# GloireLINVANI/3D_Gaussian_Splatting_Project

Hardware: AMD Instinct MI355X
Metric: Gaussians·views/sec labelled (3M G, 1080p), majority vote; first vote_view submit -> labels on the host (higher is better)
Workload: dtype f64

## Files before the change

### 3d_gaussian_splatting_project_amd/csrc/gsx_api.cpp

```cpp
#include <cstring>
#include <exception>
#include <new>

#include "gsx_ctx.hpp"

namespace gsx {

static thread_local std::string g_err;

void set_global_error(const char* fmt, ...) {
    char buf[512];
    va_list ap;
    va_start(ap, fmt);
    vsnprintf(buf, sizeof buf, fmt, ap);
    va_end(ap);
    g_err = buf;
}

int fail(Ctx* c, int code, const char* fmt, ...) {
    char buf[768];
    va_list ap;
    va_start(ap, fmt);
    vsnprintf(buf, sizeof buf, fmt, ap);
    va_end(ap);
// ... 155 lines not shown
    }
    else if (k == "render_multi_pre") c->opt_render_multi_pre = value != 0;
    else if (k == "render_bin32") c->opt_render_bin32 = value != 0;
    else if (k == "render_compact") c->opt_render_compact = value != 0;
    else if (k == "render_wide_sort") c->opt_render_wide_sort = value < 0 ? 0 : (value > 2 ? 2 : (int)value);
    else if (k == "render_share_stream") {
        if ((value != 0) != (c->opt_render_share_stream != 0)) gsx::render_release_twin(c);
        c->opt_render_share_stream = value != 0;
    }
    else if (k == "render_frames") {
        if (value < 1 || value > Ctx::kMaxFrames) return gsx::fail(c, GSX_E_INVALID, "set_option: render_frames must be in [1,%d]", (int)Ctx::kMaxFrames);
        c->opt_render_frames = (int)value;
    }
    else if (k == "blend_pk2") c->opt_blend_pk2 = value < 0 ? 0 : (value > 2 ? 2 : (int)value);
    else if (k == "exchange_slabs") {
        if (value < 1 || value > 64) return gsx::fail(c, GSX_E_INVALID, "set_option: exchange_slabs must be in [1,64]");
        c->opt_slabs = (int)value;
    } else if (k == "exchange_local") c->opt_local_codes = value != 0;
    else if (k == "flat_project") c->opt_flat_project = value != 0;
    else if (k == "seg_coarse") c->opt_seg_coarse = value != 0;
    else if (k == "batched_counts") c->opt_batched_counts = value != 0;
    else if (k == "wave_cull") c->opt_wave_cull = value != 0;
    else if (k == "filter_project") c->opt_filter_project = value != 0;
    else if (k == "host_pack") c->opt_host_pack = value != 0;
    else if (k == "labels_u8") c->opt_labels_u8 = value != 0;
    else if (k == "host_compact") c->opt_host_compact = value != 0;
    else if (k == "early_vote") {
        if (value < 0 || value > 2) return gsx::fail(c, GSX_E_INVALID, "set_option: early_vote must be 0, 1 or 2");
        c->opt_early_vote = (int)value;
    } else if (k == "early_replay") c->opt_early_replay = value != 0;
    else if (k == "early_vote_at") {
        if (value < 0 || value > 1000) return gsx::fail(c, GSX_E_INVALID, "set_option: early_vote_at must be in [0,1000] (permille of the announced views; 0 = from the hand-over rate)");
        c->opt_early_at = (int)value;
    }
    else if (k == "host_prefetch") gsx::set_host_prefetch((int)value);
    else if (k == "host_prefetch_burst") gsx::set_host_prefetch_burst(value != 0);
#ifdef GSX_EXPERIMENTS
    else if (k == "ablate") c->opt_ablate = (int)value;
#endif
    else if (k == "host_threads") {
        if (value < 0 || value > 256) return gsx::fail(c, GSX_E_INVALID, "set_option: host_threads must be in [0,256]");
        if ((int)value != c->opt_host_threads) {
            delete c->workers;
            c->workers = nullptr;
        }
        c->opt_host_threads = (int)value;
    }
    else if (k == "vote_unroll") {
        if (value != 2 && value != 4 && value != 8)
            return gsx::fail(c, GSX_E_INVALID, "set_option: vote_unroll must be 2, 4 or 8");
        c->opt_vote_unroll = (int)value;
    } else
        return gsx::fail(c, GSX_E_INVALID, "set_option: unknown option '%s'", name);
    return GSX_OK;
}

int gsx_get_option(gsx_ctx* ctx, const char* name, int64_t* value) {
    CTX_OR_FAIL(ctx);
    if (!name || !value) return gsx::fail(c, GSX_E_INVALID, "get_option: NULL argument");
    const std::string k(name);
    if (k == "early_vote") *value = c->opt_early_vote;
    else if (k == "early_vote_at") *value = c->opt_early_at;
    else if (k == "early_replay") *value = c->opt_early_replay ? 1 : 0;
    else if (k == "seg_tiled") *value = c->opt_seg_tiled ? 1 : 0;
    else if (k == "seg_coarse") *value = c->opt_seg_coarse ? 1 : 0;
    else
// ... 750 lines not shown
```

### 3d_gaussian_splatting_project_amd/csrc/gsx_ctx.hpp

```cpp
#pragma once
#include <hip/hip_runtime.h>

#include <chrono>
#include <cstdarg>
#include <cstdint>
#include <cstdio>
#include <map>
#include <cstddef>
#include <string>
#include <vector>

#include "../../include/gsx.h"
#include "host_pack.hpp"

namespace gsx {

void set_global_error(const char* fmt, ...);
struct Ctx;
int fail(Ctx* c, int code, const char* fmt, ...);

#define GSX_HIP(ctx, call)                                                                         \
    do {                                                                                           \
        hipError_t e__ = (call);                                                                   \
        if (e__ != hipSuccess)                                                                     \
// ... 161 lines not shown
    void* h_scratch = nullptr;
    size_t h_scratch_cap = 0;
    long long compact_bytes = 0;
    void* h_labels = nullptr;
    size_t h_labels_cap = 0;
    hipEvent_t h_ev[kLabelChunks] = {nullptr, nullptr, nullptr, nullptr};
    void* h_views = nullptr;
    size_t h_views_cap = 0;
    hipEvent_t h_views_ev = nullptr;
    std::vector<ViewDesc> own_views;
    int own_first_view = 0;
    const void* pool_base = nullptr;
    int n_flushed = 0;
    bool planes_valid = false;
    bool planes_zero = false;
    bool planes_stale = false;
    DevBuf cnt, fv;
    DevBuf keys, labels;
    DevBuf labels8;
    DevBuf bcnt, bcodes;
    DevBuf cand, codes;
    long long counts_n = -1, counts_npad = -1, counts_sn = -1, codes_n = -1, codes_npad = -1;
    int counts_bins = -1;
    bool labels_valid = false;
    int opt_filter_project = 1;
    int opt_early_vote = 1;
    int opt_early_at = 0;
    std::chrono::steady_clock::time_point early_t0;
    int opt_early_replay = 1;
    bool early_replayed = false;
    int early_state = 0;
    int early_done = 0;
    int early_batches = 0;
    hipStream_t stream2 = nullptr;
    bool stream_borrowed = false;
    int opt_render_share_stream = 1;
    bool early_inflight = false;
    hipEvent_t early_maps_ev = nullptr, early_done_ev = nullptr, early_up_ev = nullptr;
    DevBuf ecnt, efv;
    DevBuf erec;
    DevBuf e_views, e_cull;
    void* h_early = nullptr;
    size_t h_early_cap = 0;

    int64_t rn = 0;
    DevBuf r_order, r_buffer, r_tex;
    DevBuf r_sh;
    DevBuf r_fdc, r_shc;
    bool r_sh_valid = false, r_sh_on = false;
    int r_sh_deg = 0;
    DevBuf r_labels, r_edit_code, r_edit_tab, r_edit_hidden;
    bool r_edits_on = false;
    int64_t r_edit_hidden_n = 0;
    DevBuf r_image;
    int r_W = 0, r_H = 0;
    DevBuf r_ranges, r_small, r_scan;
    DevBuf r_depth, r_bucket, r_rect, r_count, r_offset, r_rec;
    DevBuf r_pre;
    struct PreSet {
        DevBuf depth, rect, rec, pre;
    };
    static constexpr int kPreSets = 3;
    PreSet r_sets[kPreSets];
    DevBuf r_pre_args;
    std::vector<unsigned long long> r_pre_args_host;
    hipEvent_t r_pre_ev[kPreSets] = {nullptr, nullptr, nullptr};
// ... 156 lines not shown
```

### 3d_gaussian_splatting_project_amd/csrc/vote.hip

```cpp
#include <hip/hip_runtime.h>

#include <chrono>
#include <cmath>

#include <algorithm>
#include <cmath>
#include <cstdlib>
#include <cstring>
#include <new>

#include <type_traits>

#include "gsx_ctx.hpp"

namespace gsx {

static constexpr int kBlock = 256;
static constexpr int kMaxBatch = 255;
int early_join(Ctx* c);

struct ViewRegs {
    double R[9], t[3], fx, fy, half_w, half_h, width, height;
    long long seg_off;
    int seg_w, unit_scale, seg_row_bytes, cam_w, cam_h;
// ... 490 lines not shown
    const double Z = valid ? (double)p.z[i] : 0.0;
    const uint8_t* __restrict__ pool = p.pool;

    int best = -1;
    int bestc = 0;
    const CullMasks cmask = wave_cull_masks(p.cull, p.cull_pitch, p.nviews, X, Y, Z, p.cull_tally);
    auto chunk = [&](auto full, int vb) {
        constexpr bool kFull = decltype(full)::value;
        int bin[U];
        gather_chunk<U, DIV, kFull>(views, pool, vb, X, Y, Z, cull_bits<U>(cmask, p.nviews - vb), bin, p.filt_h);
#pragma unroll
        for (int u = 0; u < U; ++u) {
            if (bin[u] >= 0) {
                const int c = h[bin[u]] + 1;
                h[bin[u]] = (uint8_t)c;
                if (c >= bestc) {
                    bestc = c;
                    best = bin[u];
                }
            }
        }
        };
    int vb = p.nviews;
    for (; vb >= U; vb -= U) chunk(std::true_type{}, vb);
    if (vb > 0) chunk(std::false_type{}, vb);
    if (valid) {
        const long long o = p.perm ? (long long)p.perm[i] : i;
        labels[o] = best - 1 + (best < 0);
    }
}

template <int U, int DIV>
__global__ __launch_bounds__(kBlock) void vote_record_kernel(FusedParams p, const ViewDesc* __restrict__ views,
                                                             uint8_t* __restrict__ rec) {
    const long long i = (long long)logical_block(blockIdx.x, gridDim.x, p.xcd_swizzle) * kBlock + threadIdx.x;
    const bool valid = i < p.n;
    const long long ic = valid ? i : 0;
    const float xf = p.x[ic], yf = p.y[ic], zf = p.z[ic];
    const double X = valid ? (double)xf : __builtin_nan("");
    const double Y = valid ? (double)yf : 0.0;
    const double Z = valid ? (double)zf : 0.0;
    const uint8_t* __restrict__ pool = p.pool;
    const int lane = threadIdx.x & 63;
    uint8_t* r = rec + (i - lane) * p.nviews + lane;
    const CullMasks cmask = wave_cull_masks(p.cull, p.cull_pitch, p.nviews, X, Y, Z, p.cull_tally);
    auto chunk = [&](auto full, int vb) {
        constexpr bool kFull = decltype(full)::value;
        int bin[U];
        gather_chunk<U, DIV, kFull>(views, pool, vb, X, Y, Z, cull_bits<U>(cmask, p.nviews - vb), bin, p.filt_h);
#pragma unroll
        for (int u = 0; u < U; ++u)
            if (kFull || vb - 1 - u >= 0) r[(vb - 1 - u) * 64] = (uint8_t)(bin[u] + 1);
    };
    int vb = p.nviews;
    for (; vb >= U; vb -= U) chunk(std::true_type{}, vb);
    if (vb > 0) chunk(std::false_type{}, vb);
}

template <int U, int DIV>
__global__ __launch_bounds__(kBlock) void vote_fused_replay_kernel(FusedParams p, const ViewDesc* __restrict__ views,
                                                                   const uint8_t* __restrict__ rec, int E,
                                                                   int* __restrict__ labels) {
    extern __shared__ uint32_t lds[];
    uint32_t* row = lds + threadIdx.x * p.stride_dw;
    uint8_t* h = reinterpret_cast<uint8_t*>(row);
    for (int k = 0; k < p.stride_dw; ++k) row[k] = 0;
    const long long i = (long long)logical_block(blockIdx.x, gridDim.x, p.xcd_swizzle) * kBlock + threadIdx.x;
    const bool valid = i < p.n;
    const long long ic = valid ? i : 0;
    const float xf = p.x[ic], yf = p.y[ic], zf = p.z[ic];
    const double X = valid ? (double)xf : __builtin_nan("");
    const double Y = valid ? (double)yf : 0.0;
    const double Z = valid ? (double)zf : 0.0;
    const uint8_t* __restrict__ pool = p.pool;
    int best = -1, bestc = 0;
    auto vote = [&](int b) {
        const int c = h[b] + 1;
        h[b] = (uint8_t)c;
        if (c >= bestc) {
            bestc = c;
            best = b;
        }
    };
    const CullMasks cmask = wave_cull_masks(p.cull, p.cull_pitch, p.nviews, X, Y, Z, p.cull_tally);
    auto chunk = [&](auto full, int vb) {
        constexpr bool kFull = decltype(full)::value;
        int bin[U];
        gather_chunk<U, DIV, kFull>(views, pool, vb, X, Y, Z, cull_bits<U>(cmask, p.nviews - vb), bin, p.filt_h);
#pragma unroll
        for (int u = 0; u < U; ++u)
            if (bin[u] >= 0) vote(bin[u]);
    };
    int vb = p.nviews;
    for (; vb >= U; vb -= U) chunk(std::true_type{}, vb);
    if (vb > 0) chunk(std::false_type{}, vb);
    constexpr int kReplay = 16;
    const int lane = threadIdx.x & 63;
    const uint8_t* __restrict__ r = rec + (i - lane) * E + lane;
    for (int v0 = E; v0 > 0; v0 -= kReplay) {
        unsigned b[kReplay];
#pragma unroll
        for (int j = 0; j < kReplay; ++j) {
            const int v = v0 - 1 - j;
            const unsigned got = r[max(v, 0) * 64];
            b[j] = v >= 0 ? got : 0u;
        }
#pragma unroll
        for (int j = 0; j < kReplay; ++j)
            if (b[j]) vote((int)b[j] - 1);
    }
    if (valid) {
        const long long o = p.perm ? (long long)p.perm[i] : i;
        labels[o] = best - 1 + (best < 0);
    }
}

typedef unsigned short u16x2 __attribute__((ext_vector_type(2)));
__device__ __forceinline__ uint32_t pk_max_u16(uint32_t a, uint32_t b) {
    return __builtin_bit_cast(uint32_t, __builtin_elementwise_max(__builtin_bit_cast(u16x2, a), __builtin_bit_cast(u16x2, b)));
}

template <int U, int DIV, int NQ>
__global__ __launch_bounds__(kBlock, 4) void vote_fused_final_kernel(FusedParams p, const ViewDesc* __restrict__ views,
                                                                     const uint8_t* __restrict__ cntA,
                                                                     const uint8_t* __restrict__ fvA,
                                                                     const uint8_t* __restrict__ recA, int E,
                                                                     int* __restrict__ labels, int ablate_arg) {
#ifdef GSX_EXPERIMENTS
    const int ablate = ablate_arg;
#else
    constexpr int ablate = 0;
// ... 508 lines not shown
        return fail(c, GSX_E_UNSUPPORTED, "vote_begin: n_classes=%d outside [1,255] (u8 seg maps)", n_classes);
    if (first_view < 0 || total_views < 1 || total_views > 65535 || first_view >= total_views)
        return fail(c, GSX_E_INVALID, "vote_begin: first_view=%d total_views=%d (need 0 <= first < total <= 65535)",
                    first_view, total_views);
    GSX_HIP(c, hipSetDevice(c->device));
    c->n_classes = n_classes;
    c->bins = n_classes + 1;
    c->first_view = first_view;
    c->total_views = total_views;
    c->local_codes = c->opt_local_codes != 0;
    c->wide = total_views > 255 && !c->local_codes;
    c->slabs = c->opt_slabs > 0 ? c->opt_slabs : 1;
    c->sn = ((c->n + c->slabs - 1) / c->slabs + 255) / 256 * 256;
    if (c->sn == 0) c->sn = 256;
    c->n_pad = c->sn * c->slabs;
    c->views.clear();
    c->pend_count = 0;
    c->compact_bytes = 0;
    c->views_dirty = true;
    c->pool_base = nullptr;
    c->seg_used = 0;
    c->n_flushed = 0;
    c->planes_valid = false;
    c->planes_zero = false;
    c->planes_stale = false;
    c->labels_valid = false;
    {
        const int rcj = early_join(c);
        if (rcj) return rcj;
    }
    c->early_state = 0;
    c->early_done = 0;
    c->early_batches = 0;
    GSX_HIP(c, c->errflag.ensure(sizeof(int)));
    GSX_HIP(c, hipMemsetAsync(c->errflag.p, 0x7f, sizeof(int), c->stream));
    c->vote_begun = true;
    return GSX_OK;
}

static int pool_reserve(Ctx* c, size_t need) {
    if (need <= c->segpool.cap) return GSX_OK;
    {
        const int rcf = vote_flush_pending(c);
        if (rcf) return rcf;
    }
    if (c->early_state == 1 || c->early_batches > 0) {
        GSX_HIP(c, hipStreamSynchronize(c->stream2));
        c->early_inflight = false;
        c->early_state = -1;
        c->early_batches = 0;
    }
    size_t cap = c->segpool.cap ? c->segpool.cap : ((size_t)64 << 20);
    while (cap < need) cap *= 2;
    void* np = nullptr;
    GSX_HIP(c, hipMalloc(&np, cap));
    if (c->seg_used) {
        hipError_t e = hipMemcpyAsync(np, c->segpool.p, c->seg_used, hipMemcpyDeviceToDevice, c->stream);
        if (e == hipSuccess) e = hipStreamSynchronize(c->stream);
        if (e != hipSuccess) {
            (void)hipFree(np);
            return fail(c, GSX_E_HIP, "seg pool growth copy failed: %s", hipGetErrorString(e));
        }
    }
    c->segpool.release();
    c->segpool.p = np;
    c->segpool.cap = cap;
// ... 26 lines not shown
        const size_t all = stride * (size_t)(c->total_views - c->first_view);
        need = std::max(need, std::min(all, (size_t)32 << 30));
    }
    return pool_reserve(c, need);
}

static void push_view(Ctx* c, const gsx_camera* cam, const MapLayout& L, size_t off, int img_w, int img_h) {
    ViewDesc vd;
    fill_view_desc(vd, cam, L.w, L.h, img_w, img_h);
    vd.seg_off = (long long)off;
    vd.seg_row_bytes = L.strip_bytes;
    vd.coarse_row_bytes = L.cstrip_bytes;
    vd.coarse_delta = (unsigned)L.coarse_off;
    c->views.push_back(vd);
    c->views_dirty = true;
    c->seg_used = off + L.map_bytes;
    c->labels_valid = false;
}

static void launch_pack(Ctx* c, const PackArgs& a, int jobs, int seg_dtype, bool vec, long long cells);

static Workers* host_workers(Ctx* c, const void* near = nullptr) {
    if (!c->workers) {
        try {
            c->workers = new Workers(c->opt_host_threads > 0 ? c->opt_host_threads : default_host_threads(), numa_node_of(near));
        } catch (...) {
            c->workers = nullptr;
        }
    }
    return c->workers;
}

static int early_vote_stage(Ctx* c);

static int vote_view_host(Ctx* c, const gsx_camera* cam, const void* seg, int seg_dtype, int seg_w, int seg_h, int img_w, int img_h) {
    MapLayout L;
    int rc = view_prologue(c, "vote_view", cam, seg, 1, seg_dtype, seg_w, seg_h, img_w, img_h, L);
    if (rc) return rc;
    if (c->opt_host_pack) {
        const size_t stride = (L.map_bytes + 255) / 256 * 256;
        constexpr int kSlots = kDmaBatch * kDmaGroups;
        const bool compact = c->opt_host_compact && L.strip_bytes && L.cstrip_bytes;
        const CompactLayout CL = compact ? compact_layout(L) : CompactLayout{};
        const size_t slot_bytes = compact ? (CL.capacity + 255) / 256 * 256 : stride;
        if (c->hring_slot != slot_bytes || !c->hring || c->hring_compact != compact) {
            if ((rc = vote_flush_pending(c))) return rc;
            for (int g = 0; g < kDmaGroups; ++g) {
                if (c->hring_busy[g]) GSX_HIP(c, hipEventSynchronize(c->hring_ev[g]));
                c->hring_busy[g] = false;
                if (!c->hring_ev[g]) GSX_HIP(c, hipEventCreateWithFlags(&c->hring_ev[g], hipEventDisableTiming));
            }
            if (c->hring_bytes < slot_bytes * kSlots) {
                if (c->hring) GSX_HIP(c, hipHostFree(c->hring));
                c->hring = nullptr;
                c->hring_bytes = 0;
                GSX_HIP(c, hipHostMalloc(&c->hring, slot_bytes * kSlots, hipHostMallocDefault));
                c->hring_bytes = slot_bytes * kSlots;
            }
            if (!compact) std::memset(c->hring, 0, slot_bytes * kSlots);
            c->hring_slot = slot_bytes;
            c->hring_compact = compact;
            c->hring_next = 0;
            c->cgrp = 0;
            c->grp_recs = 0;
        }
        const size_t off = (c->seg_used + 255) / 256 * 256;
// ... 86 lines not shown
        if (slot.cap < raw) {
            GSX_HIP(c, hipHostFree(slot.p));
            slot.p = nullptr;
            slot.cap = 0;
            GSX_HIP(c, hipHostMalloc(&slot.p, raw, hipHostMallocDefault));
            slot.cap = raw;
        }
        DevBuf& land = c->dstage[c->ring_next];
        GSX_HIP(c, land.ensure(raw));
        host_copy(host_workers(c, seg), slot.p, seg, raw);
        GSX_HIP(c, hipMemcpyAsync(land.p, slot.p, raw, hipMemcpyHostToDevice, c->stream));
        const size_t off = (c->seg_used + 255) / 256 * 256;
        PackArgs a{};
        a.src[0] = land.p;
        a.dst[0] = c->segpool.as<uint8_t>() + off;
        a.view[0] = c->first_view + (int)c->views.size();
        a.w = L.w, a.h = L.h, a.strip_bytes = L.strip_bytes, a.cstrip_bytes = L.cstrip_bytes, a.cw = L.cw, a.ch = L.ch;
        a.bins = c->bins;
        a.coarse_off = (unsigned)L.coarse_off;
        a.err = c->errflag.as<int>();
        launch_pack(c, a, 1, seg_dtype, seg_w % 4 == 0, (long long)L.cw * L.ch);
        GSX_HIP(c, hipGetLastError());
        GSX_HIP(c, hipEventRecord(slot.ev, c->stream));
        slot.busy = true;
        c->ring_next = (c->ring_next + 1) % kPinSlots;
        push_view(c, cam, L, off, img_w, img_h);
        return GSX_OK;
    }
    return GSX_OK;
}

int vote_view(Ctx* c, const gsx_camera* cam, const void* seg, int seg_dtype, int seg_w, int seg_h, int img_w, int img_h) {
    const int rc = vote_view_host(c, cam, seg, seg_dtype, seg_w, seg_h, img_w, img_h);
    return rc ? rc : early_vote_stage(c);
}

static void launch_pack(Ctx* c, const PackArgs& a, int jobs, int seg_dtype, bool vec, long long cells) {
    using K = void (*)(PackArgs);
    static const K table[4][2] = {{seg_pack_fused_kernel<int32_t, 1, false>, seg_pack_fused_kernel<int32_t, 1, true>},
                                  {seg_pack_fused_kernel<int64_t, 1, false>, seg_pack_fused_kernel<int64_t, 1, true>},
                                  {seg_pack_fused_kernel<uint8_t, 0, false>, seg_pack_fused_kernel<uint8_t, 0, true>},
                                  {seg_pack_fused_kernel<uint8_t, 1, false>, seg_pack_fused_kernel<uint8_t, 1, true>}};
    ProfScope ps(c, "seg_pack");
    hipLaunchKernelGGL(table[seg_dtype][vec ? 1 : 0], dim3(grid_for(cells), jobs), dim3(kBlock), 0, c->stream, a);
}

int vote_views_device(Ctx* c, int n, const gsx_camera* cams, const void* const* segs, int seg_dtype, int seg_w, int seg_h,
                      int img_w, int img_h) {
    if (n <= 0) return n == 0 ? GSX_OK : fail(c, GSX_E_INVALID, "vote_views_device: n < 0");
    MapLayout L;
    int rc = view_prologue(c, "vote_views_device", cams, segs, n, seg_dtype, seg_w, seg_h, img_w, img_h, L);
    if (rc) return rc;
    for (int i = 0; i < n; ++i)
        if (!segs[i]) return fail(c, GSX_E_INVALID, "vote_views_device: map %d is NULL", i);
    const size_t esz = seg_dtype == GSX_SEG_I32 ? 4 : seg_dtype == GSX_SEG_I64 ? 8 : 1;
    const long long cells = (long long)L.cw * L.ch;
    for (int i0 = 0; i0 < n; i0 += kPackBatch) {
        const int m = std::min(kPackBatch, n - i0);
        PackArgs a{};
        bool vec = seg_w % 4 == 0;
        size_t off = 0;
        for (int k = 0; k < m; ++k) {
            off = (c->seg_used + 255) / 256 * 256;
            a.src[k] = segs[i0 + k];
            a.dst[k] = c->segpool.as<uint8_t>() + off;
            a.view[k] = c->first_view + (int)c->views.size();
            vec = vec && reinterpret_cast<uintptr_t>(segs[i0 + k]) % (4 * esz) == 0;
            push_view(c, cams + i0 + k, L, off, img_w, img_h);
        }
        a.w = L.w, a.h = L.h, a.strip_bytes = L.strip_bytes, a.cstrip_bytes = L.cstrip_bytes, a.cw = L.cw, a.ch = L.ch;
        a.bins = c->bins;
        a.coarse_off = (unsigned)L.coarse_off;
        a.err = c->errflag.as<int>();
        launch_pack(c, a, m, seg_dtype, vec, cells);
        GSX_HIP(c, hipGetLastError());
    }
    return GSX_OK;
}

int vote_flush_pending(Ctx* c) {
    if (!c->pend_count) return GSX_OK;
    GSX_HIP(c, hipSetDevice(c->device));
    if (c->hring_compact) {
        const int g = c->pend_group;
        const size_t gcap = (size_t)kDmaBatch * c->hring_slot;
        GSX_HIP(c, c->cstage.ensure(gcap));
        const uint8_t* src = static_cast<uint8_t*>(c->hring) + (size_t)g * gcap;
        if (!(c->opt_ablate & 1))
            GSX_HIP(c, hipMemcpyAsync(c->cstage.as<uint8_t>() + c->pend_lo, src + c->pend_lo, c->grp_used - c->pend_lo, hipMemcpyHostToDevice,
                                      c->stream));
        GSX_HIP(c, hipEventRecord(c->hring_ev[g], c->stream));
        c->hring_busy[g] = true;
        const MapLayout& L = c->pend_L;
        const CompactLayout CL = compact_layout(L);
        ExpandArgs a{};
        for (int k = 0; k < c->pend_count; ++k) {
            a.rec[k] = c->cstage.as<uint8_t>() + c->pend_rec[k];
            a.map[k] = c->segpool.as<uint8_t>() + c->pend_map[k];
        }
        a.w = L.w, a.h = L.h, a.strip_bytes = L.strip_bytes, a.cstrip_bytes = L.cstrip_bytes, a.cw = L.cw, a.ch = L.ch;
        a.strips = (L.w + 15) / 16;
        a.table_bytes = (unsigned)CL.table_bytes, a.stream_off = (unsigned)CL.stream_off, a.coarse_off = (unsigned)L.coarse_off;
        a.fine_bytes = (unsigned)L.fine_bytes, a.map_bytes = (unsigned)L.map_bytes, a.stride = (unsigned)((L.map_bytes + 255) / 256 * 256);
        a.max_block = (unsigned)(L.cw - 1);
        if (!(c->opt_ablate & 3)) {
            ProfScope ps(c, "seg_expand");
            hipLaunchKernelGGL(seg_expand_kernel, dim3((unsigned)CL.bands, (unsigned)c->pend_count), dim3(kBlock), 0, c->stream, a);
            GSX_HIP(c, hipGetLastError());
// ... 295 lines not shown
}

int vote_rewind(Ctx* c) {
    if (!c->vote_begun) return fail(c, GSX_E_STATE, "vote_rewind before vote_begin");
    GSX_HIP(c, hipSetDevice(c->device));
    c->n_flushed = 0;
    c->labels_valid = false;
    c->early_state = -1;
    c->early_batches = 0;
    {
        const int rcj = early_join(c);
        if (rcj) return rcj;
    }
    if (c->planes_valid) {
        c->planes_valid = false;
        c->planes_zero = false;
        c->planes_stale = true;
    }
    return GSX_OK;
}

template <class K>
static int set_lds(Ctx* c, K kernel, size_t bytes) {
    if (bytes > 160 * 1024) return fail(c, GSX_E_UNSUPPORTED, "vote: %zu B of LDS per workgroup exceeds 160 KiB", bytes);
    GSX_HIP(c, hipFuncSetAttribute(reinterpret_cast<const void*>(kernel), hipFuncAttributeMaxDynamicSharedMemorySize,
                                   (int)bytes));
    return GSX_OK;
}

static constexpr int kUnroll = 8;

FusedParams fused_params(Ctx* c, int stride_bytes_per_bin);
static constexpr int kEarlyPitch = 256;
static constexpr long long kEarlyMinGaussians = 1 << 18;
static constexpr int kEarlyMinViews = 32;
static constexpr double kEarlyUsPerGaussianView = 4.4e-6;
static constexpr double kRecordUsPerGaussianView = 1.7e-6;
static constexpr size_t kEarlySlack = 64 * 260;
static constexpr size_t kEarlyCullDoubles = (size_t)kCullStride * kCullPlanes * kEarlyPitch;

static bool early_common(const Ctx* c) {
    return c->opt_early_vote && c->first_view == 0 && !c->local_codes && c->slabs == 1 && c->n_flushed == 0 && !c->pool_base &&
           c->opt_flat_project && c->n > 0 && c->bins <= 255 &&
           (c->opt_early_vote == 2 || (c->n >= kEarlyMinGaussians && c->total_views >= kEarlyMinViews));
}
static bool early_possible(const Ctx* c) { return early_common(c) && c->total_views <= kMaxBatch && !c->wide; }
static bool early_batched_possible(const Ctx* c) { return early_common(c) && c->total_views > kMaxBatch && c->opt_batched_counts; }
static int early_batch_stage(Ctx* c);
static int early_batch_count(int total) {
    const int tail = std::min(std::max(total / 16, 16), 64), body = total - tail;
    return (body + kMaxBatch - 1) / kMaxBatch + 1;
}
static void early_batch_bounds(int total, int s, int& lo, int& hi) {
    const int tail = std::min(std::max(total / 16, 16), 64), body = total - tail;
    const int Sb = (body + kMaxBatch - 1) / kMaxBatch;
    if (s >= Sb) {
        lo = body;
        hi = total;
    } else {
        lo = (int)((long long)body * s / Sb);
        hi = (int)((long long)body * (s + 1) / Sb);
    }
}

static int early_upload(Ctx* c, int lo, int hi, int block, int blocks, hipStream_t st, int* dm) {
    const size_t vbytes = sizeof(ViewDesc) * kEarlyPitch, cbytes = sizeof(double) * kEarlyCullDoubles;
    if (!c->h_early) {
        GSX_HIP(c, hipHostMalloc(&c->h_early, vbytes + cbytes, hipHostMallocDefault));
        c->h_early_cap = vbytes + cbytes;
    }
    GSX_HIP(c, c->e_views.ensure(sizeof(ViewDesc) * (size_t)std::max(kEarlyPitch, c->total_views)));
    GSX_HIP(c, c->e_cull.ensure(cbytes * (size_t)std::max(2, blocks)));
    if (!c->early_up_ev) GSX_HIP(c, hipEventCreateWithFlags(&c->early_up_ev, hipEventDisableTiming));
    else GSX_HIP(c, hipEventSynchronize(c->early_up_ev));
    ViewDesc* hv = static_cast<ViewDesc*>(c->h_early);
    double* planes = reinterpret_cast<double*>(static_cast<char*>(c->h_early) + vbytes);
    std::memset(planes, 0, cbytes);
    const long long base = (long long)reinterpret_cast<uintptr_t>(c->segpool.p);
    bool simple = true, coarse = true;
    for (int i = lo; i < hi; ++i) {
        ViewDesc& v = hv[i - lo];
        v = c->views[i];
        v.seg_off += base;
        simple = simple && v.unit_scale && v.seg_row_bytes;
        coarse = coarse && v.coarse_row_bytes;
        double pl[kCullStride * kCullPlanes];
        cull_planes(v, pl);
        for (int k = 0; k < kCullStride * kCullPlanes; ++k) planes[(size_t)k * kEarlyPitch + (i - lo)] = pl[k];
    }
    *dm = flat_div_mode(c, simple, coarse);
    if (hi > lo) GSX_HIP(c, hipMemcpyAsync(c->e_views.as<ViewDesc>() + lo, hv, sizeof(ViewDesc) * (size_t)(hi - lo), hipMemcpyHostToDevice, st));
    GSX_HIP(c, hipMemcpyAsync(c->e_cull.as<double>() + (size_t)block * kEarlyCullDoubles, planes, cbytes, hipMemcpyHostToDevice, st));
    GSX_HIP(c, hipEventRecord(c->early_up_ev, st));
    return GSX_OK;
}

static FusedParams early_params(Ctx* c, int lo, int hi, int block, int stride_bytes_per_bin) {
    FusedParams p = fused_params(c, stride_bytes_per_bin);
    p.views = c->e_views.as<ViewDesc>() + lo;
    p.nviews = hi - lo;
    p.cull = c->opt_wave_cull ? c->e_cull.as<double>() + (size_t)block * kEarlyCullDoubles : nullptr;
    p.cull_pitch = kEarlyPitch;
    return p;
}

int early_join(Ctx* c) {
    if (!c->early_inflight) return GSX_OK;
    GSX_HIP(c, hipStreamWaitEvent(c->stream, c->early_done_ev, 0));
    c->early_inflight = false;
    return GSX_OK;
}

int second_stream(Ctx* c) {
    if (c->stream2) return GSX_OK;
    int least = 0, greatest = 0;
    GSX_HIP(c, hipDeviceGetStreamPriorityRange(&least, &greatest));
    GSX_HIP(c, hipStreamCreateWithPriority(&c->stream2, hipStreamNonBlocking, least));
    return GSX_OK;
}

static int early_streams(Ctx* c) {
    const int rc = second_stream(c);
    if (rc) return rc;
    if (!c->early_maps_ev) GSX_HIP(c, hipEventCreateWithFlags(&c->early_maps_ev, hipEventDisableTiming));
    if (!c->early_done_ev) GSX_HIP(c, hipEventCreateWithFlags(&c->early_done_ev, hipEventDisableTiming));
    return GSX_OK;
}

static int early_vote_stage(Ctx* c) {
    if (c->early_state == 0 && early_batched_possible(c)) return early_batch_stage(c);
    if (c->early_state != 0 || !early_possible(c)) return GSX_OK;
    const int nv = (int)c->views.size();
    int at;
    if (c->opt_early_at > 0) {
        at = std::max(1, (int)(((long long)c->total_views * c->opt_early_at + 999) / 1000));
        if (nv != at) return GSX_OK;
    } else {
        const auto now = std::chrono::steady_clock::now();
        if (nv == 1) c->early_t0 = now;
        if (nv < std::max(8, c->total_views / 4)) return GSX_OK;
        const double t_map = std::chrono::duration<double, std::micro>(now - c->early_t0).count() / (double)(nv - 1);
        const double t_view = (c->opt_early_replay ? kRecordUsPerGaussianView : kEarlyUsPerGaussianView) * (double)c->n;
        const int lo = (c->total_views + 1) / 2, hi = (int)(((long long)c->total_views * 880) / 1000);
        const int want = std::min(std::max((int)std::ceil(c->total_views * t_map / (t_map + t_view)), lo), std::max(lo, hi));
        if (nv < want) return GSX_OK;
        at = nv;
    }
    if (at >= c->total_views) return GSX_OK;
    int rc = vote_flush_pending(c);
    if (rc) return rc;
    if ((rc = early_streams(c))) return rc;
    const size_t plane = (size_t)c->bins * (size_t)c->n_pad;
    if (!c->opt_early_replay) {
        GSX_HIP(c, c->ecnt.ensure(plane + kEarlySlack));
        GSX_HIP(c, c->efv.ensure(plane + kEarlySlack));
    }
    GSX_HIP(c, c->erec.ensure((size_t)c->n_pad * (size_t)at));
    if ((rc = ensure_tally(c))) return rc;
    GSX_HIP(c, hipEventRecord(c->early_maps_ev, c->stream));
    GSX_HIP(c, hipStreamWaitEvent(c->stream2, c->early_maps_ev, 0));
    int dm = kDivFlat;
    if ((rc = early_upload(c, 0, at, 0, 2, c->stream2, &dm))) return rc;
    if (c->opt_early_replay) {
        FusedParams p = early_params(c, 0, at, 0, 1);
        auto kr = with_div<true>(dm, [](auto d) { return vote_record_kernel<kUnroll, decltype(d)::value>; });
        {
            ProfScope ps(c, "vote_early_record", c->stream2);
            hipLaunchKernelGGL(kr, dim3(grid_for(c->n)), dim3(kBlock), 0, c->stream2, p, p.views, c->erec.as<uint8_t>());
            GSX_HIP(c, hipGetLastError());
        }
        GSX_HIP(c, hipEventRecord(c->early_done_ev, c->stream2));
        c->early_inflight = true;
        c->early_done = at;
        c->early_state = 1;
        c->early_replayed = true;
        return GSX_OK;
    }
    c->early_replayed = false;
    FusedParams p = early_params(c, 0, at, 0, 2);
    const size_t lds = (size_t)kBlock * p.stride_dw * 4;
    auto k = with_div<true>(dm, [](auto d) { return vote_fused_planes_kernel<kUnroll, uint8_t, decltype(d)::value>; });
    if ((rc = set_lds(c, k, lds))) return rc;
    {
        ProfScope ps(c, "vote_early_planes", c->stream2);
        hipLaunchKernelGGL(k, dim3(grid_for(c->n)), dim3(kBlock), lds, c->stream2, p, p.views, c->ecnt.as<uint8_t>(), c->efv.as<uint8_t>(),
                           64LL, 0, 1, 0, c->erec.as<uint8_t>());
        GSX_HIP(c, hipGetLastError());
    }
    GSX_HIP(c, hipEventRecord(c->early_done_ev, c->stream2));
    c->early_inflight = true;
    c->early_done = at;
    c->early_state = 1;
    return GSX_OK;
}

static int early_batch_stage(Ctx* c) {
    const int nv = (int)c->views.size();
    const int S = early_batch_count(c->total_views);
    const int s = c->early_batches;
    if (s >= S - 1) return GSX_OK;
    int lo, hi;
    early_batch_bounds(c->total_views, s, lo, hi);
    if (nv != hi) return GSX_OK;
    int rc = vote_flush_pending(c);
    if (rc) return rc;
    if ((rc = early_streams(c))) return rc;
    const size_t plane = (size_t)c->bins * (size_t)c->n_pad;
    GSX_HIP(c, c->bcnt.ensure(plane * S));
    if ((rc = ensure_tally(c))) return rc;
    GSX_HIP(c, hipEventRecord(c->early_maps_ev, c->stream));
    GSX_HIP(c, hipStreamWaitEvent(c->stream2, c->early_maps_ev, 0));
    int dm = kDivFlat;
    if ((rc = early_upload(c, lo, hi, s, S, c->stream2, &dm))) return rc;
    FusedParams p = early_params(c, lo, hi, s, 1);
    const size_t lds = (size_t)kBlock * p.stride_dw * 4;
    auto k = with_div<true>(dm, [](auto d) { return vote_fused_counts_kernel<kUnroll, decltype(d)::value>; });
    if ((rc = set_lds(c, k, lds))) return rc;
    {
        ProfScope ps(c, "vote_early_counts", c->stream2);
        hipLaunchKernelGGL(k, dim3(grid_for(c->n)), dim3(kBlock), lds, c->stream2, p, p.views, c->bcnt.as<uint8_t>() + plane * s, (long long)c->n_pad);
        GSX_HIP(c, hipGetLastError());
    }
    GSX_HIP(c, hipEventRecord(c->early_done_ev, c->stream2));
    c->early_inflight = true;
    c->early_batches = s + 1;
    c->early_done = hi;
    return GSX_OK;
}

static int early_vote_finish(Ctx* c) {
    const int nv = (int)c->views.size();
    int rc = vote_flush_pending(c);
    if (rc) return rc;
    int dm = kDivFlat;
    if ((rc = early_upload(c, c->early_done, nv, 1, 2, c->stream, &dm))) return rc;
    GSX_HIP(c, c->labels.ensure(sizeof(int) * (size_t)(c->n_pad ? c->n_pad : 1)));
    if (c->early_replayed) {
        FusedParams pr = early_params(c, c->early_done, nv, 1, 1);
        const size_t ldsr = (size_t)kBlock * pr.stride_dw * 4;
        auto kr = with_div<true>(dm, [](auto d) { return vote_fused_replay_kernel<kUnroll, decltype(d)::value>; });
        if ((rc = set_lds(c, kr, ldsr))) return rc;
        if ((rc = early_join(c))) return rc;
        if ((c->opt_ablate >> 4) & 2) pr.nviews = 0;
        ProfScope ps(c, "vote_fused_replay");
        hipLaunchKernelGGL(kr, dim3(grid_for(c->n)), dim3(kBlock), ldsr, c->stream, pr, pr.views, c->erec.as<uint8_t>(), c->early_done,
                           c->labels.as<int>());
        GSX_HIP(c, hipGetLastError());
        return GSX_OK;
    }
    FusedParams p = early_params(c, c->early_done, nv, 1, 1);
    const size_t lds = (size_t)(kBlock / 64) * ((c->bins + 3) / 4) * 256;
    constexpr int kRegRows = 38;
    const bool regs = c->bins <= 4 * kRegRows;
    auto k = with_div<true>(dm, [&](auto d) {
        constexpr int kDiv = decltype(d)::value;
        return regs ? vote_fused_final_kernel<kUnroll, kDiv, kRegRows> : vote_fused_final_kernel<kUnroll, kDiv, 0>;
    });
    if ((rc = set_lds(c, k, lds))) return rc;
    if ((rc = early_join(c))) return rc;
    const int ablate = (c->opt_ablate >> 4) & 63;
    if (ablate & 2) p.nviews = 0;
    ProfScope ps(c, "vote_fused_final");
    hipLaunchKernelGGL(k, dim3(grid_for(c->n)), dim3(kBlock), lds, c->stream, p, p.views, c->ecnt.as<uint8_t>(), c->efv.as<uint8_t>(),
                       c->erec.as<uint8_t>(), c->early_done, c->labels.as<int>(), ablate);
    GSX_HIP(c, hipGetLastError());
    return GSX_OK;
}

int vote_flush(Ctx* c) {
    if (!c->vote_begun) return fail(c, GSX_E_STATE, "vote_flush before vote_begin");
    GSX_HIP(c, hipSetDevice(c->device));
    int rc = early_join(c);
    if (rc) return rc;
    if ((rc = sync_views(c))) return rc;
    rc = ensure_planes(c);
    if (rc) return rc;
    const int nv = (int)c->views.size();
    if (c->n <= 0 || c->n_flushed >= nv) {
        c->n_flushed = nv;
        return clear_stale_planes(c);
    }
    FusedParams p{};
    p.x = c->x.as<float>();
// ... 231 lines not shown
    {
        ProfScope ps(c, "vote_tie_resolve");
        hipLaunchKernelGGL(vote_tie_resolve_kernel, dim3(grid_for(npad)), dim3(kBlock), 0, c->stream, c->bcodes.as<uint16_t>(), S, npad,
                           c->keys.as<int>());
    }
    GSX_HIP(c, hipGetLastError());
    return GSX_OK;
}

static int labels_for_range(Ctx* c, const VoteRange& r, bool to_sorted) {
    int rc = early_join(c);
    if (rc) return rc;
    if ((rc = sync_views(c))) return rc;
    GSX_HIP(c, c->keys.ensure(sizeof(int) * (size_t)(c->n_pad ? c->n_pad : 1)));
    GSX_HIP(c, c->labels.ensure(sizeof(int) * (size_t)(c->n_pad ? c->n_pad : 1)));
    const uint32_t* perm = c->sorted ? c->perm.as<uint32_t>() : nullptr;
    if ((int)c->views.size() <= kMaxBatch)
        return labels_one_batch(c, r, to_sorted ? nullptr : perm, to_sorted ? c->keys.as<int>() : c->labels.as<int>());
    if ((rc = labels_batched(c, r))) return rc;
    if (!to_sorted && r.n > 0) {
        ProfScope ps(c, "vote_labels");
        hipLaunchKernelGGL(unpermute_labels_kernel, dim3(grid_for(r.n)), dim3(kBlock), 0, c->stream, c->keys.as<int>(), r.n, perm,
                           c->labels.as<int>());
        GSX_HIP(c, hipGetLastError());
    }
    return GSX_OK;
}

int vote_finalize(Ctx* c, int32_t* labels_out) {
    if (!c->vote_begun) return fail(c, GSX_E_STATE, "vote_finalize before vote_begin");
    GSX_HIP(c, hipSetDevice(c->device));
    const int nv = (int)c->views.size();
    const bool batched_ok = !c->local_codes && c->opt_batched_counts;
    if (c->early_state == 1 && early_possible(c) && nv >= c->early_done && nv <= kMaxBatch) {
        int rc = early_vote_finish(c);
        if (rc) return rc;
        return labels_to_host(c, labels_out);
    }
    if (c->n_flushed == 0 && (nv <= kMaxBatch || batched_ok)) {
        int rc = labels_for_range(c, VoteRange{0, c->n}, false);
        if (rc) return rc;
        return labels_to_host(c, labels_out);
    }
    int rc = vote_flush(c);
    if (rc) return rc;
    if ((rc = vote_tiebreak_keys(c))) return rc;
    return vote_labels_from_keys(c, labels_out);
}

int vote_export(Ctx* c, int64_t reserve_bytes, void* blobs_out, void** pool_dev, int64_t* pool_bytes) {
    if (!c->vote_begun) return fail(c, GSX_E_STATE, "vote_export before vote_begin");
    if (c->pool_base) return fail(c, GSX_E_STATE, "vote_export after vote_import");
    GSX_HIP(c, hipSetDevice(c->device));
    if (reserve_bytes < 0) return fail(c, GSX_E_INVALID, "vote_export: negative size");
    {
        const int rcf = vote_flush_pending(c);
        if (rcf) return rcf;
    }
    const size_t used = (c->seg_used + 255) / 256 * 256;
    int rc = pool_reserve(c, std::max<size_t>(std::max<size_t>((size_t)reserve_bytes, used), 256));
    if (rc) return rc;
    c->views_dirty = true;
    static_assert(sizeof(ViewDesc) == GSX_VIEW_BLOB_BYTES, "view blob size is part of the ABI");
    if (blobs_out && !c->views.empty()) std::memcpy(blobs_out, c->views.data(), sizeof(ViewDesc) * c->views.size());
    if (pool_dev) *pool_dev = c->segpool.p;
    if (pool_bytes) *pool_bytes = (int64_t)used;
// ... 310 lines not shown
```

Baseline: 95.17 billion.

## Stage early vote recording incrementally as device maps arrive

Adds multi-stage early recording for the device-map path. Each batch of packed views can launch a record kernel on the side stream once enough views have accumulated, leaving a tail fraction for the final replay kernel. The record buffer now uses a fixed pitch of total_views with a row offset, and the pinned upload staging is split into several slices so stages do not wait on each other. This overlaps vote work with map ingestion, at the cost of more launches and more bookkeeping about when the path must be disabled.

```diff
diff --git a/3d_gaussian_splatting_project_amd/csrc/gsx_api.cpp b/3d_gaussian_splatting_project_amd/csrc/gsx_api.cpp
--- a/3d_gaussian_splatting_project_amd/csrc/gsx_api.cpp
+++ b/3d_gaussian_splatting_project_amd/csrc/gsx_api.cpp
@@ -211,6 +211,12 @@
     else if (k == "early_vote_at") {
         if (value < 0 || value > 1000) return gsx::fail(c, GSX_E_INVALID, "set_option: early_vote_at must be in [0,1000] (permille of the announced views; 0 = from the hand-over rate)");
         c->opt_early_at = (int)value;
+    } else if (k == "early_stage_views") {
+        if (value < 1 || value > 255) return gsx::fail(c, GSX_E_INVALID, "set_option: early_stage_views must be in [1,255] (device maps: views per record stage)");
+        c->opt_early_stage_views = (int)value;
+    } else if (k == "early_tail") {
+        if (value < 0 || value > 1000) return gsx::fail(c, GSX_E_INVALID, "set_option: early_tail must be in [0,1000] (device maps: permille of the announced views left to the last stage)");
+        c->opt_early_tail = (int)value;
     }
     else if (k == "host_prefetch") gsx::set_host_prefetch((int)value);
     else if (k == "host_prefetch_burst") gsx::set_host_prefetch_burst(value != 0);
diff --git a/3d_gaussian_splatting_project_amd/csrc/gsx_ctx.hpp b/3d_gaussian_splatting_project_amd/csrc/gsx_ctx.hpp
--- a/3d_gaussian_splatting_project_amd/csrc/gsx_ctx.hpp
+++ b/3d_gaussian_splatting_project_amd/csrc/gsx_ctx.hpp
@@ -217,6 +217,13 @@
     int early_state = 0;
     int early_done = 0;
     int early_batches = 0;
+    int opt_early_stage_views = 48;
+    int opt_early_tail = 450;
+    int early_stages = 0;
+    int early_dev_views = 0;
+    bool early_dev = false;
+    bool early_dev_ok = true;
+    int early_geo[4] = {0, 0, 0, 0};
     hipStream_t stream2 = nullptr;
     bool stream_borrowed = false;
     int opt_render_share_stream = 1;
diff --git a/3d_gaussian_splatting_project_amd/csrc/vote.hip b/3d_gaussian_splatting_project_amd/csrc/vote.hip
--- a/3d_gaussian_splatting_project_amd/csrc/vote.hip
+++ b/3d_gaussian_splatting_project_amd/csrc/vote.hip
@@ -546,7 +546,7 @@
 
 template <int U, int DIV>
 __global__ __launch_bounds__(kBlock) void vote_record_kernel(FusedParams p, const ViewDesc* __restrict__ views,
-                                                             uint8_t* __restrict__ rec) {
+                                                             uint8_t* __restrict__ rec, int pitch, int row0) {
     const long long i = (long long)logical_block(blockIdx.x, gridDim.x, p.xcd_swizzle) * kBlock + threadIdx.x;
     const bool valid = i < p.n;
     const long long ic = valid ? i : 0;
@@ -556,7 +556,7 @@
     const double Z = valid ? (double)zf : 0.0;
     const uint8_t* __restrict__ pool = p.pool;
     const int lane = threadIdx.x & 63;
-    uint8_t* r = rec + (i - lane) * p.nviews + lane;
+    uint8_t* r = rec + (i - lane) * pitch + row0 * 64 + lane;
     const CullMasks cmask = wave_cull_masks(p.cull, p.cull_pitch, p.nviews, X, Y, Z, p.cull_tally);
     auto chunk = [&](auto full, int vb) {
         constexpr bool kFull = decltype(full)::value;
@@ -573,7 +573,7 @@
 
 template <int U, int DIV>
 __global__ __launch_bounds__(kBlock) void vote_fused_replay_kernel(FusedParams p, const ViewDesc* __restrict__ views,
-                                                                   const uint8_t* __restrict__ rec, int E,
+                                                                   const uint8_t* __restrict__ rec, int E, int pitch,
                                                                    int* __restrict__ labels) {
     extern __shared__ uint32_t lds[];
     uint32_t* row = lds + threadIdx.x * p.stride_dw;
@@ -610,7 +610,7 @@
     if (vb > 0) chunk(std::false_type{}, vb);
     constexpr int kReplay = 16;
     const int lane = threadIdx.x & 63;
-    const uint8_t* __restrict__ r = rec + (i - lane) * E + lane;
+    const uint8_t* __restrict__ r = rec + (i - lane) * pitch + lane;
     for (int v0 = E; v0 > 0; v0 -= kReplay) {
         unsigned b[kReplay];
 #pragma unroll
@@ -1185,6 +1185,10 @@
     c->early_state = 0;
     c->early_done = 0;
     c->early_batches = 0;
+    c->early_stages = 0;
+    c->early_dev_views = 0;
+    c->early_dev = false;
+    c->early_dev_ok = true;
     GSX_HIP(c, c->errflag.ensure(sizeof(int)));
     GSX_HIP(c, hipMemsetAsync(c->errflag.p, 0x7f, sizeof(int), c->stream));
     c->vote_begun = true;
@@ -1277,6 +1281,8 @@
 }
 
 static int early_vote_stage(Ctx* c);
+static int early_device_stage(Ctx* c);
+static void early_device_off(Ctx* c);
 
 static int vote_view_host(Ctx* c, const gsx_camera* cam, const void* seg, int seg_dtype, int seg_w, int seg_h, int img_w, int img_h) {
     MapLayout L;
@@ -1429,6 +1435,7 @@
 
 int vote_view(Ctx* c, const gsx_camera* cam, const void* seg, int seg_dtype, int seg_w, int seg_h, int img_w, int img_h) {
     const int rc = vote_view_host(c, cam, seg, seg_dtype, seg_w, seg_h, img_w, img_h);
+    if (!rc && c->early_dev_views) early_device_off(c);
     return rc ? rc : early_vote_stage(c);
 }
 
@@ -1452,6 +1459,9 @@
         if (!segs[i]) return fail(c, GSX_E_INVALID, "vote_views_device: map %d is NULL", i);
     const size_t esz = seg_dtype == GSX_SEG_I32 ? 4 : seg_dtype == GSX_SEG_I64 ? 8 : 1;
     const long long cells = (long long)L.cw * L.ch;
+    const int geo[4] = {seg_w, seg_h, img_w, img_h};
+    if (c->views.empty()) std::memcpy(c->early_geo, geo, sizeof geo);
+    if ((int)c->views.size() != c->early_dev_views || std::memcmp(c->early_geo, geo, sizeof geo) != 0) early_device_off(c);
     for (int i0 = 0; i0 < n; i0 += kPackBatch) {
         const int m = std::min(kPackBatch, n - i0);
         PackArgs a{};
@@ -1471,6 +1481,8 @@
         a.err = c->errflag.as<int>();
         launch_pack(c, a, m, seg_dtype, vec, cells);
         GSX_HIP(c, hipGetLastError());
+        c->early_dev_views += m;
+        if ((rc = early_device_stage(c))) return rc;
     }
     return GSX_OK;
 }
@@ -1832,6 +1844,8 @@
 
 FusedParams fused_params(Ctx* c, int stride_bytes_per_bin);
 static constexpr int kEarlyPitch = 256;
+static constexpr int kEarlyStages = 4;
+static constexpr int kEarlyBlocks = kEarlyStages + 1;
 static constexpr long long kEarlyMinGaussians = 1 << 18;
 static constexpr int kEarlyMinViews = 32;
 static constexpr double kEarlyUsPerGaussianView = 4.4e-6;
@@ -1866,15 +1880,16 @@
 static int early_upload(Ctx* c, int lo, int hi, int block, int blocks, hipStream_t st, int* dm) {
     const size_t vbytes = sizeof(ViewDesc) * kEarlyPitch, cbytes = sizeof(double) * kEarlyCullDoubles;
     if (!c->h_early) {
-        GSX_HIP(c, hipHostMalloc(&c->h_early, vbytes + cbytes, hipHostMallocDefault));
-        c->h_early_cap = vbytes + cbytes;
+        GSX_HIP(c, hipHostMalloc(&c->h_early, (vbytes + cbytes) * kEarlyBlocks, hipHostMallocDefault));
+        c->h_early_cap = (vbytes + cbytes) * kEarlyBlocks;
     }
     GSX_HIP(c, c->e_views.ensure(sizeof(ViewDesc) * (size_t)std::max(kEarlyPitch, c->total_views)));
-    GSX_HIP(c, c->e_cull.ensure(cbytes * (size_t)std::max(2, blocks)));
+    GSX_HIP(c, c->e_cull.ensure(cbytes * (size_t)std::max(kEarlyBlocks, blocks)));
     if (!c->early_up_ev) GSX_HIP(c, hipEventCreateWithFlags(&c->early_up_ev, hipEventDisableTiming));
-    else GSX_HIP(c, hipEventSynchronize(c->early_up_ev));
-    ViewDesc* hv = static_cast<ViewDesc*>(c->h_early);
-    double* planes = reinterpret_cast<double*>(static_cast<char*>(c->h_early) + vbytes);
+    else if (block == 0 || block >= kEarlyBlocks) GSX_HIP(c, hipEventSynchronize(c->early_up_ev));
+    char* slice = static_cast<char*>(c->h_early) + (vbytes + cbytes) * (size_t)(block % kEarlyBlocks);
+    ViewDesc* hv = reinterpret_cast<ViewDesc*>(slice);
+    double* planes = reinterpret_cast<double*>(slice + vbytes);
     std::memset(planes, 0, cbytes);
     const long long base = (long long)reinterpret_cast<uintptr_t>(c->segpool.p);
     bool simple = true, coarse = true;
@@ -1925,6 +1940,47 @@
     if (!c->early_maps_ev) GSX_HIP(c, hipEventCreateWithFlags(&c->early_maps_ev, hipEventDisableTiming));
     if (!c->early_done_ev) GSX_HIP(c, hipEventCreateWithFlags(&c->early_done_ev, hipEventDisableTiming));
     return GSX_OK;
+}
+
+static int early_record_stage(Ctx* c, int lo, int hi) {
+    int rc = early_streams(c);
+    if (rc) return rc;
+    GSX_HIP(c, c->erec.ensure((size_t)c->n_pad * (size_t)c->total_views));
+    if ((rc = ensure_tally(c))) return rc;
+    GSX_HIP(c, hipEventRecord(c->early_maps_ev, c->stream));
+    GSX_HIP(c, hipStreamWaitEvent(c->stream2, c->early_maps_ev, 0));
+    int dm = kDivFlat;
+    if ((rc = early_upload(c, lo, hi, c->early_stages, kEarlyBlocks, c->stream2, &dm))) return rc;
+    FusedParams p = early_params(c, lo, hi, c->early_stages, 1);
+    auto kr = with_div<true>(dm, [](auto d) { return vote_record_kernel<kUnroll, decltype(d)::value>; });
+    {
+        ProfScope ps(c, "vote_early_record", c->stream2);
+        hipLaunchKernelGGL(kr, dim3(grid_for(c->n)), dim3(kBlock), 0, c->stream2, p, p.views, c->erec.as<uint8_t>(), c->total_views, lo);
+        GSX_HIP(c, hipGetLastError());
+    }
+    GSX_HIP(c, hipEventRecord(c->early_done_ev, c->stream2));
+    c->early_inflight = true;
+    c->early_done = hi;
+    c->early_state = 1;
+    c->early_replayed = true;
+    c->early_stages += 1;
+    return GSX_OK;
+}
+
+static void early_device_off(Ctx* c) {
+    c->early_dev_ok = false;
+    if (c->early_dev && c->early_state == 1) c->early_state = -1;
+}
+
+static int early_device_stage(Ctx* c) {
+    if (!c->early_dev_ok || c->early_state < 0 || !c->opt_early_replay || !early_possible(c)) return GSX_OK;
+    if (c->early_state == 1 && !c->early_dev) return GSX_OK;
+    const int nv = (int)c->views.size();
+    const int lo = c->early_state == 1 ? c->early_done : 0;
+    const int tail = (int)(((long long)c->total_views * c->opt_early_tail + 999) / 1000);
+    if (c->early_stages >= kEarlyStages || nv - lo < c->opt_early_stage_views || c->total_views - nv < tail) return GSX_OK;
+    c->early_dev = true;
+    return early_record_stage(c, lo, nv);
 }
 
 static int early_vote_stage(Ctx* c) {
@@ -1955,28 +2011,15 @@
         GSX_HIP(c, c->ecnt.ensure(plane + kEarlySlack));
         GSX_HIP(c, c->efv.ensure(plane + kEarlySlack));
     }
+    if (c->opt_early_replay) return early_record_stage(c, 0, at);
     GSX_HIP(c, c->erec.ensure((size_t)c->n_pad * (size_t)at));
     if ((rc = ensure_tally(c))) return rc;
     GSX_HIP(c, hipEventRecord(c->early_maps_ev, c->stream));
     GSX_HIP(c, hipStreamWaitEvent(c->stream2, c->early_maps_ev, 0));
     int dm = kDivFlat;
-    if ((rc = early_upload(c, 0, at, 0, 2, c->stream2, &dm))) return rc;
-    if (c->opt_early_replay) {
-        FusedParams p = early_params(c, 0, at, 0, 1);
-        auto kr = with_div<true>(dm, [](auto d) { return vote_record_kernel<kUnroll, decltype(d)::value>; });
-        {
-            ProfScope ps(c, "vote_early_record", c->stream2);
-            hipLaunchKernelGGL(kr, dim3(grid_for(c->n)), dim3(kBlock), 0, c->stream2, p, p.views, c->erec.as<uint8_t>());
-            GSX_HIP(c, hipGetLastError());
-        }
-        GSX_HIP(c, hipEventRecord(c->early_done_ev, c->stream2));
-        c->early_inflight = true;
-        c->early_done = at;
-        c->early_state = 1;
-        c->early_replayed = true;
-        return GSX_OK;
-    }
+    if ((rc = early_upload(c, 0, at, 0, kEarlyBlocks, c->stream2, &dm))) return rc;
     c->early_replayed = false;
+    c->early_stages = 1;
     FusedParams p = early_params(c, 0, at, 0, 2);
     const size_t lds = (size_t)kBlock * p.stride_dw * 4;
     auto k = with_div<true>(dm, [](auto d) { return vote_fused_planes_kernel<kUnroll, uint8_t, decltype(d)::value>; });
@@ -2033,10 +2076,11 @@
     int rc = vote_flush_pending(c);
     if (rc) return rc;
     int dm = kDivFlat;
-    if ((rc = early_upload(c, c->early_done, nv, 1, 2, c->stream, &dm))) return rc;
+    const int block = c->early_stages;
+    if ((rc = early_upload(c, c->early_done, nv, block, kEarlyBlocks, c->stream, &dm))) return rc;
     GSX_HIP(c, c->labels.ensure(sizeof(int) * (size_t)(c->n_pad ? c->n_pad : 1)));
     if (c->early_replayed) {
-        FusedParams pr = early_params(c, c->early_done, nv, 1, 1);
+        FusedParams pr = early_params(c, c->early_done, nv, block, 1);
         const size_t ldsr = (size_t)kBlock * pr.stride_dw * 4;
         auto kr = with_div<true>(dm, [](auto d) { return vote_fused_replay_kernel<kUnroll, decltype(d)::value>; });
         if ((rc = set_lds(c, kr, ldsr))) return rc;
@@ -2044,11 +2088,11 @@
         if ((c->opt_ablate >> 4) & 2) pr.nviews = 0;
         ProfScope ps(c, "vote_fused_replay");
         hipLaunchKernelGGL(kr, dim3(grid_for(c->n)), dim3(kBlock), ldsr, c->stream, pr, pr.views, c->erec.as<uint8_t>(), c->early_done,
-                           c->labels.as<int>());
+                           c->total_views, c->labels.as<int>());
         GSX_HIP(c, hipGetLastError());
         return GSX_OK;
     }
-    FusedParams p = early_params(c, c->early_done, nv, 1, 1);
+    FusedParams p = early_params(c, c->early_done, nv, block, 1);
     const size_t lds = (size_t)(kBlock / 64) * ((c->bins + 3) / 4) * 256;
     constexpr int kRegRows = 38;
     const bool regs = c->bins <= 4 * kRegRows;
@@ -2346,6 +2390,7 @@
     GSX_HIP(c, hipSetDevice(c->device));
     const int nv = (int)c->views.size();
     const bool batched_ok = !c->local_codes && c->opt_batched_counts;
+    if (c->early_state == 1 && c->early_dev && nv != c->total_views) c->early_state = -1;
     if (c->early_state == 1 && early_possible(c) && nv >= c->early_done && nv <= kMaxBatch) {
         int rc = early_vote_finish(c);
         if (rc) return rc;
```

New measurement: 89.22 billion. 6.3% lower.
